# rvaser/rala

Measured on AMD Instinct MI355X. Metric: overlaps/sec (pile build + transitive reduction), higher is better.
Workload: dtype u16/u32 (+f64 compares)

## Files before the change

include/rala_hip.h:

```cpp
#ifndef RALA_HIP_H_
#define RALA_HIP_H_

#include <stddef.h>
#include <stdint.h>

#ifdef __cplusplus
extern "C" {
#endif

#define RALA_HIP_NO_READ 0xFFFFFFFFu

enum {
    RALA_HIP_OK = 0,
    RALA_HIP_EDEVICE = -1,
    RALA_HIP_EINVAL = -2,
    RALA_HIP_ECAPACITY = -3,
    RALA_HIP_EFILTERED = -4,
    RALA_HIP_ENOMEM = -5,
    RALA_HIP_ENOTAFILE = -6,
    RALA_HIP_ETOOLARGE = -7
};

enum { RALA_HIP_TYPE_X = 0, RALA_HIP_TYPE_A = 1, RALA_HIP_TYPE_B = 2, RALA_HIP_TYPE_AB = 3, RALA_HIP_TYPE_BA = 4 };

// ... 169 lines not shown

int rala_hip_get_valid(rala_hip_ctx* ctx, uint8_t* valid);
int rala_hip_get_piles(rala_hip_ctx* ctx, uint32_t* begin, uint32_t* end, uint16_t* median, uint16_t* p10,
                       uint8_t* alive);
int rala_hip_get_pile_data(rala_hip_ctx* ctx, uint64_t read, uint16_t* data);
int rala_hip_get_pile_row_digests(rala_hip_ctx* ctx, uint64_t* fnv, uint64_t* inside, uint64_t* outside);
int rala_hip_get_pile_rows_info(rala_hip_ctx* ctx, uint64_t* resident_bytes, uint64_t* rows_materialised);
int rala_hip_get_intervals(rala_hip_ctx* ctx, int kind, uint64_t* offsets, uint32_t* pairs, uint32_t* aux);
int rala_hip_get_overlaps(rala_hip_ctx* ctx, int which, uint64_t* n, uint32_t* src_index, uint32_t* a_begin,
                          uint32_t* a_end, uint32_t* b_begin, uint32_t* b_end, uint32_t* length, uint8_t* type);
int rala_hip_get_graph_size(rala_hip_ctx* ctx, uint64_t* n_nodes, uint64_t* n_edges);
int rala_hip_get_graph(rala_hip_ctx* ctx, uint32_t* node_read, uint32_t* src, uint32_t* dst, uint32_t* len,
                       uint8_t* marks);
int rala_hip_get_timings(rala_hip_ctx* ctx, rala_hip_timings* out);
int rala_hip_get_num_prefiltered(rala_hip_ctx* ctx, uint64_t* n);

#ifdef __cplusplus
}
#endif

#endif
```

rala_amd/csrc/kernels.h:

```cpp
#pragma once

#include <hip/hip_runtime.h>
#include <stdint.h>

#include "gzip_types.h"

namespace rala_hip {

constexpr uint32_t kPadL = 848;

enum : uint32_t {
    kErrRegionCapacity = 1u,
    kErrPoolCapacity = 2u,
    kErrRawCapacity = 4u,
};

struct Interval {
    uint32_t first, second;
    uint32_t aux;
};

struct PileArgs {
    const uint32_t* read_len;
    const uint64_t* pile_off;
// ... 250 lines not shown
    uint32_t* counts;
};
void launch_sens_split(const uint32_t* list, uint32_t bound, const uint32_t* n_dev, const SensSplitArgs& args, hipStream_t s);
void launch_status_clear(uint32_t* status, uint32_t bits, uint32_t* zero, hipStream_t s);
void launch_scatter_component_medians(const uint32_t* alive_reads, const uint8_t* touched, const uint16_t* cmed, uint32_t n_alive,
                                      uint16_t* out, hipStream_t s);
void launch_break_hills(const TailReads& R, uint32_t n_reads, hipStream_t s);
void launch_break_pits(const TailReads& R, const uint32_t* alive_reads, const uint8_t* touched, const uint16_t* comp_median,
                       uint32_t n_alive, hipStream_t s, const uint32_t* gate = nullptr);
void launch_retrim(const TailList& L, const TailReads& R, uint32_t promote, uint32_t round, uint32_t* dropped,
                   hipStream_t s, const uint32_t* gate = nullptr);
void launch_cc_edges(const TailList& L, const uint32_t* rank, uint32_t* edges, uint8_t* touched, uint32_t* label, uint32_t n_labels,
                     hipStream_t s);
void launch_refresh_types(const TailList& L, const TailReads& R, hipStream_t s);
hipError_t launch_tail_contain(const TailList& L, const TailReads& R, uint8_t* alive, uint32_t* const lists[6], uint32_t* zeroed21, uint32_t* const work[4],
                               uint32_t* base2, uint8_t* mark2, uint32_t* map, uint32_t* pack, uint32_t n_reads, uint32_t lds_limit, uint32_t debug_give_up, hipStream_t s);
void launch_count_zero_u8(const uint8_t* x, uint32_t n, uint32_t* out, hipStream_t s);
void launch_tail_init(const TailList& L, uint32_t n0, const TailReads& R, uint32_t* n_pits0, uint32_t n_reads, uint32_t* base2,
                      uint8_t* mark2, uint32_t* map, uint32_t* zero22, hipStream_t s);
struct ScanSpace;
bool launch_rank_pass(const uint8_t* alive, uint32_t* rank, uint32_t* alive_reads, uint32_t n_reads, ScanSpace& space, hipStream_t s);
bool launch_node_pass(const uint8_t* alive, uint32_t* node_rank, uint32_t* node_read, uint32_t* n_final, uint32_t n_reads,
                      ScanSpace& space, hipStream_t s);
bool launch_segment_pass(const TailList& L, const TailReads& R, uint32_t want_state, uint32_t want_round, uint32_t* base,
                         uint32_t* next, uint32_t* kept_item, const uint32_t* node_rank, uint32_t* e_src, uint32_t* e_dst,
                         uint32_t* e_len, ScanSpace& space, hipStream_t s);
bool launch_offsets_pass(const uint32_t* in, uint32_t* out, uint32_t* copy, uint32_t n, ScanSpace& space, hipStream_t s);
bool launch_pair_offsets_pass(const uint32_t* in0, const uint32_t* in1, uint32_t* out0, uint32_t* out1, uint32_t* totals, uint32_t n,
                              ScanSpace& space, hipStream_t s);

struct FixedPointList {
// ... 145 lines not shown
uint32_t gzip_segment_bytes();
uint32_t gzip_ring_symbols();
uint32_t gzip_crc_of_segments(const uint32_t* seg_crc, uint64_t text_n);
void launch_gzip_carry(uint16_t* sym, const uint8_t* text, uint64_t text_n, uint16_t* tmp, hipStream_t s);
uint32_t gzip_crc_register(const uint32_t* seg_crc, uint64_t text_n);
uint32_t gzip_crc_chain(const uint32_t* reg, const uint64_t* len, uint64_t n);
uint32_t gzip_crc_register_chain(const uint32_t* reg, const uint64_t* len, uint64_t n);

size_t scan_workspace_bytes(uint64_t n);
void launch_exclusive_scan(const uint32_t* in, uint32_t* out, uint64_t n, void* workspace, hipStream_t s);

void launch_tr_mark(const uint32_t* row_ptr, const uint32_t* adj_edge, const uint32_t* edge_src,
                    const uint32_t* edge_dst, const uint32_t* edge_len, uint32_t n_nodes, uint32_t first_edge,
                    uint32_t last_edge, uint8_t* marks, hipStream_t s);
void launch_tr_degree(const uint32_t* src, const uint32_t* dst, uint32_t n_nodes, uint32_t n_edges, uint32_t* deg,
                      uint32_t* bad, hipStream_t s);
void launch_tr_fill(const uint32_t* src, const uint32_t* dst, uint32_t n_nodes, uint32_t n_edges, uint32_t* cursor, uint32_t* adj,
                    hipStream_t s);
void launch_cc_init(uint32_t* label, uint32_t n, hipStream_t s);
void launch_cc_hook(const uint32_t* edges, uint32_t n_edges, uint32_t sample, uint32_t* label, uint32_t* changed,
                    hipStream_t s);
void launch_cc_compress(uint32_t* label, uint32_t n, hipStream_t s);
void launch_cc_compress_count(uint32_t* label, uint32_t n, const uint8_t* touched, uint32_t* size, hipStream_t s);
size_t component_median_workspace(uint32_t n);
void component_median_clear(void* tmp, uint32_t n, FillList& fills);
uint32_t* component_median_sizes(void* tmp, uint32_t n);
hipError_t launch_component_medians(const uint32_t* label, const uint8_t* touched, const uint32_t* alive_reads,
                                    const uint16_t* median, uint32_t n_alive, void* tmp, uint16_t* cmed, hipStream_t s);
void launch_tr_count(uint8_t* marks, uint32_t n_edges, uint32_t* n_pairs, hipStream_t s);

void launch_layout_step(uint32_t n, const double* x, const double* y, double* x_out, double* y_out,
                        const uint32_t* adj_off, const uint32_t* adj, double k, double t, hipStream_t s);

// ... 2 lines not shown
```

rala_amd/csrc/pipeline.hip:

```cpp
#include <hip/hip_runtime.h>
#include <stdio.h>
#include <stdlib.h>
#include <string.h>

#include <algorithm>
#include <chrono>
#include <numeric>

#include "context.h"
#include "scan_pass.h"
#include "stages.h"

using namespace rala_hip;


hipError_t rala_hip::d2h_small(rala_hip_ctx* ctx, void* dst, const void* src, size_t bytes, hipStream_t s) {
    if (ctx->p_stage.ensure(256) != hipSuccess || ctx->stage_used + bytes > 256 * sizeof(uint32_t) ||
        ctx->stage_pending.size() >= 16) {
        return hipMemcpyAsync(dst, src, bytes, hipMemcpyDeviceToHost, s);
    }
    char* at = (char*)ctx->p_stage.p + ctx->stage_used;
    const hipError_t e = hipMemcpyAsync(at, src, bytes, hipMemcpyDeviceToHost, s);
    if (e != hipSuccess) return e;
    ctx->stage_pending.push_back({dst, ctx->stage_used, bytes});
// ... 1192 lines not shown
    DevBuf<uint32_t>* B = ctx->d_tr;
    HIPCHECK(B[0].ensure(n_nodes + 2)); HIPCHECK(B[1].ensure(n_nodes + 2)); HIPCHECK(B[2].ensure(2 * (size_t)n_edges));
    HIPCHECK(ctx->d_tr_marks.ensure((size_t)n_edges + 8));
    HIPCHECK(ctx->d_scan_ws.ensure(scan_workspace_bytes((uint64_t)n_nodes + 2)));
    HIPCHECK(hipEventRecord(ctx->ev[10], s));
    FillList fills;
    fills.add(ctx->d_tr_marks.p, 0, ((size_t)n_edges + 7) & ~(size_t)3);
    fills.add(ctx->d_small.p + 2, 0, 8);
    fills.add(B[1].p, 0, (size_t)(n_nodes + 1) * 4);
    ScanSpace sp;
    {
        const int rc = scan_space(ctx, 1, n_nodes, sp, &fills);
        if (rc != RALA_HIP_OK) return rc;
    }
    HIPCHECK(fills.launch(s));
    launch_tr_degree(d_src, d_dst, n_nodes, n_edges, B[1].p, ctx->d_small.p + 2, s);
    HIPCHECK(B[3 + 3].ensure(n_nodes + 2));
    if (!launch_offsets_pass(B[1].p, B[0].p, B[6].p, n_nodes, sp, s)) return fail(ctx, RALA_HIP_EDEVICE, "scan space");
    launch_tr_fill(d_src, d_dst, n_nodes, n_edges, B[6].p, B[2].p, s);
    if (!comm) {
        launch_tr_mark(B[0].p, B[2].p, d_src, d_dst, d_len, n_nodes, 0, n_edges, ctx->d_tr_marks.p, s);
    } else {
        const uint64_t P = comm->world(), k = comm->rank();
        launch_tr_mark(B[0].p, B[2].p, d_src, d_dst, d_len, n_nodes, (uint32_t)(n_edges * k / P), (uint32_t)(n_edges * (k + 1) / P),
                       ctx->d_tr_marks.p, s);
        if (comm->all_reduce_u32((uint32_t*)ctx->d_tr_marks.p, ((size_t)n_edges + 3) / 4, ReduceOp::kSum, s) != 0) {
            ctx->err = std::string("all-reduce of the transitive marks: ") + comm->error();
            return RALA_HIP_EDEVICE;
        }
    }
    launch_tr_count(ctx->d_tr_marks.p, n_edges, ctx->d_small.p + 3, s);
    HIPCHECK(hipEventRecord(ctx->ev[11], s));
    uint32_t res[2] = {0, 0};
    HIPCHECK(d2h_small(ctx, res, ctx->d_small.p + 2, 8, s));
// ... 51 lines not shown
    else HIPCHECK(hipMemsetAsync(ctx->d_scan_state.p, 0, words * 8, ctx->stream));
    return RALA_HIP_OK;
}

int tail_components(rala_hip_ctx* ctx, const TailList& L, uint32_t n_alive, bool touched_cleared) {
    hipStream_t s = ctx->stream;
    const uint32_t M = L.n;
    if (!touched_cleared) {
        FillList fills;
        fills.add(ctx->d_touched.p, 0, n_alive);
        component_median_clear(ctx->d_med_tmp.p, n_alive, fills);
        HIPCHECK(fills.launch(s));
    }
    launch_cc_edges(L, ctx->d_rank.p, ctx->d_cc_edges.p, ctx->d_touched.p, ctx->d_cc_label.p, n_alive, s);
    for (int k = 0; k < 2; ++k) {
        launch_cc_hook(ctx->d_cc_edges.p, M, 1, ctx->d_cc_label.p, ctx->d_cc_flags.p + 7, s);
        launch_cc_compress(ctx->d_cc_label.p, n_alive, s);
    }
    launch_cc_hook(ctx->d_cc_edges.p, M, 0, ctx->d_cc_label.p, ctx->d_cc_flags.p + 7, s);
    launch_cc_compress_count(ctx->d_cc_label.p, n_alive, ctx->d_touched.p, component_median_sizes(ctx->d_med_tmp.p, n_alive), s);
    HIPCHECK(launch_component_medians(ctx->d_cc_label.p, ctx->d_touched.p, ctx->d_alive_reads.p, ctx->d_median.p, n_alive,
                                      ctx->d_med_tmp.p, ctx->d_cmed.p, s));
    return RALA_HIP_OK;
}

int gpu_tail_part_a(rala_hip_ctx* ctx) {
    hipStream_t s = ctx->stream;
    Trace trc;
    auto mark = [&](const char* what, size_t k = 0) {
        if (trc.on) { (void)stream_sync(ctx, s); trc(what, k); }
    };
// ... 32 lines not shown
    HIPCHECK(ctx->d_fp_pack.ensure(fixed_point_pack_words()));
    launch_tail_init(L, ctx->t_n0, R, ctx->d_n_pits0.p, n_reads, ctx->d_t_fin.p, ctx->d_t_mark.p, ctx->d_fp_map.p, ctx->d_counts.p + 9, s);
    if (!launch_rank_pass(ctx->d_alive.p, ctx->d_rank.p, ctx->d_alive_reads.p, n_reads, sp, s)) return fail(ctx, RALA_HIP_EDEVICE, "scan space");
    mark("tail: ranks", n_alive);

    HIPCHECK(ctx->d_counts.ensure(48));
    uint32_t* dropped = ctx->d_counts.p + 4;
    launch_break_hills(R, n_reads, s);
    if (ctx->lists_pending) {
        HIPCHECK(hipStreamWaitEvent(s, ctx->ev[3], 0));
        ctx->lists_pending = false;
    }
    launch_retrim(L, R, 0, 0, dropped, s);
    mark("tail: hills + retrim", M);

    uint32_t rounds = 0;
    for (;;) {
        const uint32_t batch = rounds == 0 ? 2u : 1u;
        for (uint32_t k = 0; k < batch; ++k) {
            if (rounds + k >= 255) return fail(ctx, RALA_HIP_EDEVICE, "chimera loop did not settle");
            const uint32_t* gate = k ? dropped + k - 1 : nullptr;
            FillList fills;
            fills.add(ctx->d_dirty.p, 0, n_reads);
            fills.add(ctx->d_touched.p, 0, n_alive);
            component_median_clear(ctx->d_med_tmp.p, n_alive, fills);
            if (k == 0) fills.add(dropped, 0, 2 * 4);
            HIPCHECK(fills.launch(s));
            const int rcc = tail_components(ctx, L, n_alive, true);
            if (rcc != RALA_HIP_OK) return rcc;
            launch_break_pits(R, ctx->d_alive_reads.p, ctx->d_touched.p, ctx->d_cmed.p, n_alive, s, gate);
            launch_retrim(L, R, 1, rounds + k, dropped + k, s, gate);
        }
        uint32_t d[2] = {0, 0};
        HIPCHECK(d2h_small(ctx, d, dropped, sizeof(d), s));
        HIPCHECK(stream_sync(ctx, s));
        mark("tail: pits + retrim", d[0] + d[1]);
        if (!d[0]) { rounds += 1; break; }
        rounds += batch;
        if (!d[batch - 1]) break;
    }
    ctx->t_rounds = rounds;
    if ((uint64_t)M * ((uint64_t)rounds + 2ull) >= 0xFFFFFFF0ull) {
        return fail(ctx, RALA_HIP_ETOOLARGE, "too many surviving overlaps for 32-bit list positions");
    }

    {
        uint32_t* const work[4] = {ctx->d_t_death[0].p, ctx->d_t_death[1].p, ctx->d_t_work[0].p, ctx->d_t_work[1].p};
        uint32_t* const lists[6] = {ctx->d_kill[0].p, ctx->d_kill[1].p, ctx->d_kill[2].p, ctx->d_kill2[0].p, ctx->d_kill2[1].p,
                                    ctx->d_kill2[2].p};
        HIPCHECK(launch_tail_contain(L, R, ctx->d_alive.p, lists, ctx->d_counts.p + 9, work, ctx->d_t_fin.p, ctx->d_t_mark.p, ctx->d_fp_map.p,
                                     ctx->d_fp_pack.p, n_reads, ctx->debug_fp_lds_limit, ctx->debug_fp_give_up, s));
    }
    mark("tail: containment scans", M);
    return RALA_HIP_OK;
}

int gpu_tail_part_b(rala_hip_ctx* ctx) {
    hipStream_t s = ctx->stream;
    Trace trc;
    auto mark = [&](const char* what, size_t k = 0) {
        if (trc.on) { (void)stream_sync(ctx, s); trc(what, k); }
    };
    const uint32_t n_reads = (uint32_t)ctx->n_reads;
    const uint32_t M = ctx->t_n0 + ctx->t_n1;
    const TailList L = tail_list(ctx);
    const TailReads R = tail_reads(ctx);
    const uint32_t n_seg = ctx->t_rounds + 1;
// ... 1765 lines not shown

int rala_hip_get_timings(rala_hip_ctx* ctx, rala_hip_timings* out) {
    if (!ctx || !out) return RALA_HIP_EINVAL;
    *out = ctx->tm;
    out->total_ms = ctx->tm.dedupe_ms + ctx->tm.bucket_ms + ctx->tm.pile_ms + ctx->tm.classify_ms + ctx->tm.death_ms +
                    ctx->tm.finish_ms + ctx->tm.tail_host_ms + ctx->tm.tr_ms;
    return RALA_HIP_OK;
}

int rala_hip_get_num_prefiltered(rala_hip_ctx* ctx, uint64_t* n) {
    if (!ctx || !n) return RALA_HIP_EINVAL;
    *n = ctx->n_prefiltered;
    return RALA_HIP_OK;
}

}
```

rala_amd/csrc/tail_kernels.hip:

```cpp
#include <hip/hip_runtime.h>

#include <algorithm>

#include "device_utils.h"
#include "geom.h"
#include "kernels.h"
#include "scan_pass.h"

namespace rala_hip {

namespace {

constexpr int kBlock = 256;
constexpr uint32_t kInf = 0xFFFFFFFFu;

inline dim3 grid_for(uint64_t n) { return dim3((unsigned)((n + kBlock - 1) / kBlock)); }

__device__ __forceinline__ bool dev_shrink(const TailReads& R, uint32_t r, uint32_t b, uint32_t e) {
    if (b > e || e - b < kMinRegion) { R.dirty[r] = 1; return false; }
    if (R.begin[r] != b || R.end[r] != e) R.dirty[r] = 1;
    R.begin[r] = b;
    R.end[r] = e;
    return true;
}
// ... 129 lines not shown
        if (m) {
            const uint32_t leader = (uint32_t)__ffsll((long long)m) - 1u;
            if (lane == leader) base = atomicAdd(s_cnt, (uint32_t)__popcll(m));
            base = (uint32_t)__shfl((int)base, (int)leader);
        }
        return mine ? base + (uint32_t)__popcll(m & ((1ull << lane) - 1ull)) : kInf;
    }
    __device__ void reserve(uint32_t* counter) const {
        __syncthreads();
        if (threadIdx.x == 0) *s_base = *s_cnt ? atomicAdd(counter, *s_cnt) : 0u;
        __syncthreads();
    }
};

__global__ __launch_bounds__(kContainBlock) void tail_contain_collect_kernel(TailList L, TailReads R, const uint8_t* __restrict__ alive,
                                                                             TailKillers K) {
    __shared__ uint32_t s_cnt[2], s_base[2];
    if (threadIdx.x < 2) s_cnt[threadIdx.x] = 0;
    __syncthreads();
    const BlockAppend app[2] = {{&s_cnt[0], &s_base[0]}, {&s_cnt[1], &s_base[1]}};
    uint32_t key[kCollectPer], target[kCollectPer], keeper[kCollectPer], slot[kCollectPer], cls[kCollectPer];
#pragma unroll
    for (uint32_t u = 0; u < kCollectPer; ++u) {
        const uint32_t k = (blockIdx.x * kCollectPer + u) * kContainBlock + threadIdx.x;
        bool killer = false;
        cls[u] = 0; key[u] = 0; target[u] = 0; keeper[u] = 0;
        if (k < L.n) {
            const uint8_t st = L.state[k];
            uint8_t t = L.type[k];
            if (st != 0 && t == 255) {
                const uint32_t a = L.a[k], b = L.b[k];
// ... 21 lines not shown
    app[1].reserve(&K.count[1]);
#pragma unroll
    for (uint32_t u = 0; u < kCollectPer; ++u) {
        if (slot[u] == kInf) continue;
        const uint32_t at = cls[u] ? L.n - 1u - (s_base[1] + slot[u]) : s_base[0] + slot[u];
        K.key[at] = key[u]; K.target[at] = target[u]; K.keeper[at] = keeper[u];
        K.mark[cls[u]][target[u]] = 1;
    }
}

__device__ __forceinline__ bool gone_before_second_scan(const uint8_t* alive, const uint32_t* base0, uint32_t r) {
    return !alive[r] || base0[r] != kInf;
}

template <int kClass>
__global__ __launch_bounds__(kBlock) void tail_contain_reduce_kernel(TailKillers K, uint32_t n_items, const uint8_t* __restrict__ alive) {
    __shared__ uint32_t s_cnt, s_base;
    const BlockAppend app = {&s_cnt, &s_base};
    const uint32_t n = K.count[kClass];
    uint32_t* base = K.base[kClass];
    for (uint32_t i0 = blockIdx.x * kBlock; i0 < n; i0 += gridDim.x * kBlock) {
        if (threadIdx.x == 0) s_cnt = 0;
        __syncthreads();
        const uint32_t i = i0 + threadIdx.x;
        bool conditional = false;
        uint32_t key = 0, target = 0, keeper = 0;
        if (i < n) {
            const uint32_t at = kClass ? n_items - 1u - i : i;
            key = K.key[at]; target = K.target[at]; keeper = K.keeper[at];
            const bool ok = kClass == 0 || !(gone_before_second_scan(alive, K.base[0], target) ||
                                             gone_before_second_scan(alive, K.base[0], keeper));
// ... 2 lines not shown
                else if (ld_past_l1(base + target) > key) atomicMin(base + target, key);
            }
        }
        const uint32_t slot = app.note(conditional);
        app.reserve(&K.count[2 + kClass]);
        if (conditional) {
            const uint32_t w = s_base + slot;
            K.c_key[w] = key; K.c_target[w] = target; K.c_keeper[w] = keeper;
        }
        __syncthreads();
    }
}

__global__ __launch_bounds__(kBlock) void tail_contain_apply_kernel(TailList L, const uint8_t* __restrict__ alive,
                                                                    const uint32_t* __restrict__ base0,
                                                                    const uint32_t* __restrict__ base1) {
    const uint32_t k = blockIdx.x * kBlock + threadIdx.x;
    if (k >= L.n) return;
    const uint8_t st = L.state[k];
    if (st == 0) return;
    const uint8_t t = L.type[k];
    bool drop = t == kTypeA || t == kTypeB;
    if (st == 2 && !drop) {
        const uint32_t a = L.a[k], b = L.b[k];
        drop = gone_before_second_scan(alive, base0, a) || gone_before_second_scan(alive, base0, b) || base1[a] < k || base1[b] < k;
    }
    if (drop) L.state[k] = 0;
}

__global__ __launch_bounds__(kBlock) void tail_contain_kill_kernel(TailKillers K, uint32_t n_items, uint8_t* alive) {
    const uint32_t n0 = K.count[0], n1 = K.count[1];
    for (uint32_t i = blockIdx.x * kBlock + threadIdx.x; i < n0 + n1; i += gridDim.x * kBlock) {
        const uint32_t target = K.target[i < n0 ? i : n_items - 1u - (i - n0)];
        if (K.base[0][target] != kInf || K.base[1][target] != kInf) alive[target] = 0;
    }
}

__global__ __launch_bounds__(kBlock) void tail_init_kernel(uint8_t* state, uint8_t* round, uint32_t n0, uint32_t m,
                                                           uint8_t* dirty, uint32_t* n_pits0, const uint32_t* n_pits,
                                                           uint32_t n_reads, uint32_t* base2, uint8_t* mark2, uint32_t* map, uint32_t* zero22) {
    const uint32_t k = blockIdx.x * kBlock + threadIdx.x;
    if (k < 22) zero22[k] = 0;
    if (k < n_reads) {
        base2[k] = kInf; base2[n_reads + k] = kInf; map[k] = kInf;
        mark2[k] = 0; mark2[n_reads + k] = 0;
// ... 115 lines not shown
    }
}
void launch_retrim(const TailList& L, const TailReads& R, uint32_t promote, uint32_t round, uint32_t* dropped,
                   hipStream_t s, const uint32_t* gate) {
    if (L.n) hipLaunchKernelGGL(retrim_kernel, grid_for(L.n), dim3(kBlock), 0, s, L, R, promote, round, dropped, gate);
}
void launch_cc_edges(const TailList& L, const uint32_t* rank, uint32_t* edges, uint8_t* touched, uint32_t* label, uint32_t n_labels,
                     hipStream_t s) {
    const uint32_t n = std::max<uint32_t>(L.n, n_labels);
    if (n) hipLaunchKernelGGL(cc_edges_kernel, grid_for(n), dim3(kBlock), 0, s, L, rank, edges, touched, label, n_labels);
}
void launch_refresh_types(const TailList& L, const TailReads& R, hipStream_t s) {
    if (L.n) hipLaunchKernelGGL(refresh_types_kernel, grid_for(L.n), dim3(kBlock), 0, s, L, R);
}
hipError_t launch_tail_contain(const TailList& L, const TailReads& R, uint8_t* alive, uint32_t* const lists[6], uint32_t* zeroed21, uint32_t* const work[4],
                               uint32_t* base2, uint8_t* mark2, uint32_t* map, uint32_t* pack, uint32_t n_reads, uint32_t lds_limit, uint32_t debug_give_up, hipStream_t s) {
    if (!L.n) return hipSuccess;
    TailKillers K;
    K.key = lists[0]; K.target = lists[1]; K.keeper = lists[2];
    K.c_key = lists[3]; K.c_target = lists[4]; K.c_keeper = lists[5];
    K.error = zeroed21; K.count = zeroed21 + 1;
    K.mark[0] = mark2; K.mark[1] = mark2 + n_reads;
    K.base[0] = base2; K.base[1] = base2 + n_reads;
    const uint32_t per_block = kCollectPer * kContainBlock;
    hipLaunchKernelGGL(tail_contain_collect_kernel, dim3((L.n + per_block - 1) / per_block), dim3(kContainBlock), 0, s, L, R,
                       (const uint8_t*)alive, K);
    for (int c = 0; c < 2; ++c) {
        if (c == 0) hipLaunchKernelGGL(tail_contain_reduce_kernel<0>, dim3(128), dim3(kBlock), 0, s, K, L.n, (const uint8_t*)alive);
        else hipLaunchKernelGGL(tail_contain_reduce_kernel<1>, dim3(128), dim3(kBlock), 0, s, K, L.n, (const uint8_t*)alive);
        const FixedPointList conditional = {K.c_key, K.c_target, K.c_keeper, K.count + 2 + c, lds_limit, debug_give_up};
        const hipError_t e = launch_fixed_point_finish(conditional, K.base[c], map, pack, work, zeroed21 + 5 + 8 * c, K.error, nullptr, s);
        if (e != hipSuccess) return e;
    }
    hipLaunchKernelGGL(tail_contain_apply_kernel, grid_for(L.n), dim3(kBlock), 0, s, L, (const uint8_t*)alive,
                       (const uint32_t*)K.base[0], (const uint32_t*)K.base[1]);
    hipLaunchKernelGGL(tail_contain_kill_kernel, dim3(128), dim3(kBlock), 0, s, K, L.n, alive);
    return hipGetLastError();
}
void launch_tail_init(const TailList& L, uint32_t n0, const TailReads& R, uint32_t* n_pits0, uint32_t n_reads, uint32_t* base2,
                      uint8_t* mark2, uint32_t* map, uint32_t* zero22, hipStream_t s) {
    const uint32_t n = std::max<uint32_t>(std::max<uint32_t>(L.n, n_reads), 22u);
    hipLaunchKernelGGL(tail_init_kernel, grid_for(n), dim3(kBlock), 0, s, L.state, L.round, n0, L.n, R.dirty, n_pits0, R.n_pits, n_reads,
                       base2, mark2, map, zero22);
}
bool launch_rank_pass(const uint8_t* alive, uint32_t* rank, uint32_t* alive_reads, uint32_t n_reads, ScanSpace& space, hipStream_t s) {
    return launch_scan_pass(n_reads, RankPass{alive, rank, alive_reads}, space, s);
}
bool launch_node_pass(const uint8_t* alive, uint32_t* node_rank, uint32_t* node_read, uint32_t* n_final, uint32_t n_reads,
                      ScanSpace& space, hipStream_t s) {
    return launch_scan_pass(n_reads, NodePass{alive, node_rank, node_read, n_final}, space, s);
}
// ... 29 lines not shown
```

rala_amd/csrc/tr_kernels.hip:

```cpp
#include <hip/hip_runtime.h>

#include "device_utils.h"
#include "geom.h"
#include "kernels.h"

namespace rala_hip {

namespace {

constexpr int kBlock = 256;

__global__ __launch_bounds__(kBlock) void tr_mark_kernel(const uint32_t* __restrict__ row_ptr,
                                                         const uint2* __restrict__ adj,
                                                         const uint32_t* __restrict__ esrc,
                                                         const uint32_t* __restrict__ edst,
                                                         const uint32_t* __restrict__ elen, uint32_t n_nodes,
                                                         uint32_t first_edge, uint32_t n_edges, uint8_t* marks) {
    const uint32_t e_ab = first_edge + blockIdx.x * kBlock + threadIdx.x;
    if (e_ab >= n_edges) return;
    const uint32_t a = esrc[e_ab], b = edst[e_ab];
    if (a >= n_nodes || b >= n_nodes) return;
    const uint32_t len_ab = elen[e_ab];
    const uint32_t a0 = row_ptr[a], a1 = row_ptr[a + 1];
    const uint32_t b0 = row_ptr[b], b1 = row_ptr[b + 1];
// ... 37 lines not shown
}

__global__ __launch_bounds__(kBlock) void tr_count_kernel(uint8_t* __restrict__ marks, uint32_t n_edges,
                                                          uint32_t* n_pairs) {
    __shared__ uint32_t tmp[kBlock / 64 + 1];
    uint32_t v = 0;
    for (uint32_t p = blockIdx.x * kBlock + threadIdx.x; 2 * p + 1 < n_edges; p += gridDim.x * kBlock) {
        if (marks[2 * p]) { marks[2 * p] = 1; marks[2 * p + 1] = 1; ++v; }
    }
    v = block_reduce<kBlock>(v, OpAdd(), 0u, tmp);
    if (threadIdx.x == 0 && v) atomicAdd(n_pairs, v);
}

__global__ __launch_bounds__(kBlock) void tr_degree_kernel(const uint32_t* __restrict__ src,
                                                           const uint32_t* __restrict__ dst, uint32_t n_nodes,
                                                           uint32_t n_edges, uint32_t* deg, uint32_t* bad) {
    const uint32_t e = blockIdx.x * kBlock + threadIdx.x;
    if (e >= n_edges) return;
    const uint32_t a = src[e], b = dst[e];
    if (a >= n_nodes || b >= n_nodes) { *bad = 1; return; }
    atomicAdd(&deg[a], 1u);
}

__global__ __launch_bounds__(kBlock) void tr_fill_kernel(const uint32_t* __restrict__ src, const uint32_t* __restrict__ dst,
                                                         uint32_t n_nodes, uint32_t n_edges, uint32_t* cursor, uint2* adj) {
    const uint32_t e = blockIdx.x * kBlock + threadIdx.x;
    if (e >= n_edges) return;
    const uint32_t a = src[e];
    if (a >= n_nodes) return;
    adj[atomicAdd(&cursor[a], 1u)] = make_uint2(e, dst[e]);
}

__global__ __launch_bounds__(kBlock) void cc_init_kernel(uint32_t* label, uint32_t n) {
    const uint32_t v = blockIdx.x * kBlock + threadIdx.x;
    if (v < n) label[v] = v;
}

__device__ __forceinline__ uint32_t cc_root(const uint32_t* label, uint32_t v) {
    uint32_t p = label[v];
    while (p != v) { v = p; p = label[v]; }
    return v;
}

__global__ __launch_bounds__(kBlock) void cc_hook_kernel(const uint32_t* __restrict__ edges, uint32_t n_edges,
                                                         uint32_t sample, uint32_t* label, uint32_t* changed) {
    const uint32_t e = blockIdx.x * kBlock + threadIdx.x;
    bool hooked = false;
    if (e < n_edges) {
        const uint32_t a = edges[2 * e], b = edges[2 * e + 1];
        if (a != b && (!sample || e < 2 || edges[2 * (e - 2)] != a)) {
            uint32_t ra = cc_root(label, a), rb = cc_root(label, b);
            while (ra != rb) {
                const uint32_t hi = ra > rb ? ra : rb, lo = ra > rb ? rb : ra;
                uint32_t old = __hip_atomic_load(&label[hi], __ATOMIC_RELAXED, __HIP_MEMORY_SCOPE_AGENT);
                if (old == hi) {
                    old = atomicMin(&label[hi], lo);
                    hooked = true;
                    if (old == hi) break;
                }
                ra = cc_root(label, old < lo ? old : lo);
                rb = cc_root(label, old < lo ? lo : old);
            }
        }
    }
    if (__ballot(hooked) != 0 && (threadIdx.x & 63) == 0) *changed = 1;
// ... 33 lines not shown
    if (threadIdx.x == 0) {
        uint32_t c = 0;
        for (int w = 0; w < kBlock / 64; ++w) c += s_cnt[w];
        atomicAdd(&size[shared], c);
    }
    if (t && !same) atomicAdd(&size[r], 1u);
}

}

void launch_cc_compress_count(uint32_t* label, uint32_t n, const uint8_t* touched, uint32_t* size, hipStream_t s) {
    if (n) hipLaunchKernelGGL(cc_compress_count_kernel, dim3((n + kBlock - 1) / kBlock), dim3(kBlock), 0, s, label, n, touched, size);
}

void launch_tr_degree(const uint32_t* src, const uint32_t* dst, uint32_t n_nodes, uint32_t n_edges, uint32_t* deg,
                      uint32_t* bad, hipStream_t s) {
    if (n_edges) {
        hipLaunchKernelGGL(tr_degree_kernel, dim3((n_edges + kBlock - 1) / kBlock), dim3(kBlock), 0, s, src, dst,
                           n_nodes, n_edges, deg, bad);
    }
}
void launch_tr_fill(const uint32_t* src, const uint32_t* dst, uint32_t n_nodes, uint32_t n_edges, uint32_t* cursor, uint32_t* adj,
                    hipStream_t s) {
    if (n_edges) {
        hipLaunchKernelGGL(tr_fill_kernel, dim3((n_edges + kBlock - 1) / kBlock), dim3(kBlock), 0, s, src, dst, n_nodes,
                           n_edges, cursor, (uint2*)adj);
    }
}
void launch_cc_init(uint32_t* label, uint32_t n, hipStream_t s) {
    if (n) hipLaunchKernelGGL(cc_init_kernel, dim3((n + kBlock - 1) / kBlock), dim3(kBlock), 0, s, label, n);
}
void launch_cc_hook(const uint32_t* edges, uint32_t n_edges, uint32_t sample, uint32_t* label, uint32_t* changed,
                    hipStream_t s) {
    if (n_edges) {
        hipLaunchKernelGGL(cc_hook_kernel, dim3((n_edges + kBlock - 1) / kBlock), dim3(kBlock), 0, s, edges, n_edges,
                           sample, label, changed);
    }
}
void launch_cc_compress(uint32_t* label, uint32_t n, hipStream_t s) {
    if (n) hipLaunchKernelGGL(cc_compress_kernel, dim3((n + kBlock - 1) / kBlock), dim3(kBlock), 0, s, label, n);
}
// ... 18 lines not shown
```

rala_amd/hip.py:

```python
import ctypes
import os

import numpy as np

from . import build as _build

TYPE_X, TYPE_A, TYPE_B, TYPE_AB, TYPE_BA = range(5)
NO_READ = 0xFFFFFFFF
MEM_HOST, MEM_DEVICE, MEM_HOST_ASYNC = 0, 1, 2

ERRORS = {0: "OK", -1: "EDEVICE", -2: "EINVAL", -3: "ECAPACITY", -4: "EFILTERED", -5: "ENOMEM", -6: "ENOTAFILE", -7: "ETOOLARGE"}

LIB_PATH = os.path.join(os.path.dirname(os.path.abspath(__file__)), "csrc", "librala_hip.so")

SYMBOLS = (
    "rala_hip_create", "rala_hip_destroy", "rala_hip_last_error", "rala_hip_set_option", "rala_hip_stream",
    "rala_hip_set_reads", "rala_hip_set_overlaps", "rala_hip_initialize", "rala_hip_construct",
    "rala_hip_remove_transitive_edges", "rala_hip_tr_mark", "rala_hip_get_valid", "rala_hip_get_piles",
    "rala_hip_get_pile_data", "rala_hip_get_pile_row_digests", "rala_hip_get_pile_rows_info", "rala_hip_get_intervals", "rala_hip_get_overlaps", "rala_hip_get_graph_size",
    "rala_hip_get_graph", "rala_hip_get_timings", "rala_hip_get_num_prefiltered",
    "rala_hip_dedupe", "rala_hip_emit_bound_tuples", "rala_hip_set_bound_tuples", "rala_hip_import_state",
    "rala_hip_emit_bound_tuples_bucketed", "rala_hip_get_device_state", "rala_hip_import_state_device",
    "rala_hip_bound_records_fit", "rala_hip_emit_bound_records_bucketed", "rala_hip_set_bound_records",
    "rala_hip_copy_device_state", "rala_hip_layout", "rala_hip_find_repetitive_hills",
    "rala_hip_mg_unique_id", "rala_hip_mg_local_group_create", "rala_hip_mg_local_group_destroy", "rala_hip_mg_create",
    "rala_hip_mg_create_contexts", "rala_hip_mg_join", "rala_hip_set_name_table", "rala_hip_set_overlaps_from_paf", "rala_hip_set_overlaps_from_mhap",
    "rala_hip_get_ingest_timings", "rala_hip_get_inflate_timings", "rala_hip_get_gzip_timings", "rala_hip_gzip_head", "rala_hip_gzip_chain", "rala_hip_gzip_chain_members", "rala_hip_gzip_find_members", "rala_hip_get_gzip_members", "rala_hip_bgzf_index", "rala_hip_get_overlap_columns", "rala_hip_tokenise_sensitive_paf",
    "rala_hip_mg_set_overlaps_from_paf", "rala_hip_mg_get_slice",
    "rala_hip_index_sequences", "rala_hip_get_sequence_index", "rala_hip_get_sequence_timings",
    "rala_hip_slice_sequences", "rala_hip_get_sequence_slice_info", "rala_hip_crc32_chain",
    "rala_hip_mg_destroy", "rala_hip_mg_last_error", "rala_hip_mg_set_reads", "rala_hip_mg_slice_cuts",
    "rala_hip_mg_set_overlaps", "rala_hip_mg_run", "rala_hip_mg_run_threads", "rala_hip_mg_context",
    "rala_hip_mg_owner_context",
    "rala_hip_mg_get_pile_data", "rala_hip_mg_get_pile_row_digests", "rala_hip_mg_get_timings",
)
# ... 83 lines not shown
        L.rala_hip_initialize.argtypes = [vp]
        L.rala_hip_construct.argtypes = [vp, ctypes.POINTER(OverlapsC), u64]
        L.rala_hip_remove_transitive_edges.argtypes = [vp, ctypes.POINTER(u32)]
        L.rala_hip_tr_mark.argtypes = [vp, u32, u32, vp, vp, vp, vp, ctypes.POINTER(u32)]
        L.rala_hip_get_valid.argtypes = [vp, vp]
        L.rala_hip_get_piles.argtypes = [vp, vp, vp, vp, vp, vp]
        L.rala_hip_get_pile_data.argtypes = [vp, u64, vp]
        L.rala_hip_get_pile_row_digests.argtypes = [vp, vp, vp, vp]
        L.rala_hip_get_pile_rows_info.argtypes = [vp, vp, vp]
        L.rala_hip_get_intervals.argtypes = [vp, i32, vp, vp, vp]
        L.rala_hip_get_overlaps.argtypes = [vp, i32, ctypes.POINTER(u64), vp, vp, vp, vp, vp, vp, vp]
        L.rala_hip_get_graph_size.argtypes = [vp, ctypes.POINTER(u64), ctypes.POINTER(u64)]
        L.rala_hip_get_graph.argtypes = [vp, vp, vp, vp, vp, vp]
        L.rala_hip_get_timings.argtypes = [vp, ctypes.POINTER(Timings)]
        L.rala_hip_get_num_prefiltered.argtypes = [vp, ctypes.POINTER(u64)]
        L.rala_hip_dedupe.argtypes = [vp]
        L.rala_hip_emit_bound_tuples.argtypes = [vp, vp]
        L.rala_hip_set_bound_tuples.argtypes = [vp, vp, u64, i32]
        L.rala_hip_import_state.argtypes = [vp] + [vp] * 11
        L.rala_hip_emit_bound_tuples_bucketed.argtypes = [vp, u32, vp, vp]
        L.rala_hip_get_device_state.argtypes = [vp, ctypes.POINTER(DeviceState)]
        L.rala_hip_import_state_device.argtypes = [vp, ctypes.POINTER(DeviceState)]
        L.rala_hip_copy_device_state.argtypes = [vp, ctypes.POINTER(DeviceState)]
        L.rala_hip_layout.argtypes = [vp, u32, vp, vp, vp, vp, u32, ctypes.c_double, ctypes.c_double, ctypes.c_double]
        L.rala_hip_find_repetitive_hills.argtypes = [vp, u64, u32, u32, ctypes.c_uint16, ctypes.c_uint16, ctypes.c_uint16]
        L.rala_hip_mg_unique_id.argtypes = [vp]
        L.rala_hip_mg_local_group_create.argtypes = [u32, ctypes.POINTER(vp)]
        L.rala_hip_mg_local_group_destroy.argtypes = [vp]
        L.rala_hip_mg_local_group_destroy.restype = None
        L.rala_hip_mg_create.argtypes = [i32, u32, u32, i32, vp, ctypes.POINTER(vp)]
# ... 379 lines not shown
        self._check(self.L.rala_hip_get_graph(self.h, d["node_read"].ctypes.data, d["src"].ctypes.data,
                                              d["dst"].ctypes.data, d["len"].ctypes.data,
                                              d["marked"].ctypes.data))
        return d

    def timings(self):
        t = Timings()
        self._check(self.L.rala_hip_get_timings(self.h, ctypes.byref(t)))
        return t.as_dict()

    def num_prefiltered(self):
        n = ctypes.c_uint64(0)
        self._check(self.L.rala_hip_get_num_prefiltered(self.h, ctypes.byref(n)))
        return int(n.value)


def slice_cuts(a_id, world, b_id=None):
    a = np.ascontiguousarray(a_id, dtype=np.uint32)
    b = None if b_id is None else np.ascontiguousarray(b_id, dtype=np.uint32)
    cuts = np.zeros(world + 1, dtype=np.uint64)
    rc = lib().rala_hip_mg_slice_cuts(a.ctypes.data if len(a) else None, b.ctypes.data if b is not None and len(b) else None,
                                      len(a), world, cuts.ctypes.data)
    if rc != 0:
        raise RalaHipError(rc, "slice_cuts")
    return [int(c) for c in cuts]


def unique_id():
    buf = ctypes.create_string_buffer(128)
    rc = lib().rala_hip_mg_unique_id(buf)
# ... 187 lines not shown
```

Baseline: 7.157 billion.

## Speculate containment scans ahead of retrim sync, slot-based CSR fill, cheap first hook

Containment scans are now enqueued speculatively before the host syncs on the first pits/retrim round. They are gated on a device flag, so the kernels exit early if further rounds are needed, and the scan is skipped later when it already ran. The transitive-reduction CSR fill records each edge's slot during the degree atomic, replacing the second atomic-cursor pass and the cursor copy in the offsets scan. The first connected-components hook pass uses a single relaxed load plus atomicMin instead of root chasing. A tail-rounds getter is added; the costs are extra edge-sized slot storage and possibly wasted speculative launches.

```diff
diff --git a/include/rala_hip.h b/include/rala_hip.h
--- a/include/rala_hip.h
+++ b/include/rala_hip.h
@@ -207,6 +207,7 @@
                        uint8_t* marks);
 int rala_hip_get_timings(rala_hip_ctx* ctx, rala_hip_timings* out);
 int rala_hip_get_num_prefiltered(rala_hip_ctx* ctx, uint64_t* n);
+int rala_hip_get_tail_rounds(rala_hip_ctx* ctx, uint32_t* rounds);
 
 #ifdef __cplusplus
 }
diff --git a/rala_amd/csrc/kernels.h b/rala_amd/csrc/kernels.h
--- a/rala_amd/csrc/kernels.h
+++ b/rala_amd/csrc/kernels.h
@@ -288,7 +288,8 @@
                      hipStream_t s);
 void launch_refresh_types(const TailList& L, const TailReads& R, hipStream_t s);
 hipError_t launch_tail_contain(const TailList& L, const TailReads& R, uint8_t* alive, uint32_t* const lists[6], uint32_t* zeroed21, uint32_t* const work[4],
-                               uint32_t* base2, uint8_t* mark2, uint32_t* map, uint32_t* pack, uint32_t n_reads, uint32_t lds_limit, uint32_t debug_give_up, hipStream_t s);
+                               uint32_t* base2, uint8_t* mark2, uint32_t* map, uint32_t* pack, uint32_t n_reads, uint32_t lds_limit, uint32_t debug_give_up, hipStream_t s,
+                               const uint32_t* closed = nullptr);
 void launch_count_zero_u8(const uint8_t* x, uint32_t n, uint32_t* out, hipStream_t s);
 void launch_tail_init(const TailList& L, uint32_t n0, const TailReads& R, uint32_t* n_pits0, uint32_t n_reads, uint32_t* base2,
                       uint8_t* mark2, uint32_t* map, uint32_t* zero22, hipStream_t s);
@@ -464,9 +465,9 @@
                     const uint32_t* edge_dst, const uint32_t* edge_len, uint32_t n_nodes, uint32_t first_edge,
                     uint32_t last_edge, uint8_t* marks, hipStream_t s);
 void launch_tr_degree(const uint32_t* src, const uint32_t* dst, uint32_t n_nodes, uint32_t n_edges, uint32_t* deg,
-                      uint32_t* bad, hipStream_t s);
-void launch_tr_fill(const uint32_t* src, const uint32_t* dst, uint32_t n_nodes, uint32_t n_edges, uint32_t* cursor, uint32_t* adj,
-                    hipStream_t s);
+                      uint32_t* slot, uint32_t* bad, hipStream_t s);
+void launch_tr_fill(const uint32_t* src, const uint32_t* dst, uint32_t n_nodes, uint32_t n_edges, const uint32_t* row_ptr,
+                    const uint32_t* slot, uint32_t* adj, hipStream_t s);
 void launch_cc_init(uint32_t* label, uint32_t n, hipStream_t s);
 void launch_cc_hook(const uint32_t* edges, uint32_t n_edges, uint32_t sample, uint32_t* label, uint32_t* changed,
                     hipStream_t s);
diff --git a/rala_amd/csrc/pipeline.hip b/rala_amd/csrc/pipeline.hip
--- a/rala_amd/csrc/pipeline.hip
+++ b/rala_amd/csrc/pipeline.hip
@@ -1230,10 +1230,10 @@
         if (rc != RALA_HIP_OK) return rc;
     }
     HIPCHECK(fills.launch(s));
-    launch_tr_degree(d_src, d_dst, n_nodes, n_edges, B[1].p, ctx->d_small.p + 2, s);
-    HIPCHECK(B[3 + 3].ensure(n_nodes + 2));
-    if (!launch_offsets_pass(B[1].p, B[0].p, B[6].p, n_nodes, sp, s)) return fail(ctx, RALA_HIP_EDEVICE, "scan space");
-    launch_tr_fill(d_src, d_dst, n_nodes, n_edges, B[6].p, B[2].p, s);
+    HIPCHECK(B[3 + 3].ensure(n_edges));
+    launch_tr_degree(d_src, d_dst, n_nodes, n_edges, B[1].p, B[6].p, ctx->d_small.p + 2, s);
+    if (!launch_offsets_pass(B[1].p, B[0].p, nullptr, n_nodes, sp, s)) return fail(ctx, RALA_HIP_EDEVICE, "scan space");
+    launch_tr_fill(d_src, d_dst, n_nodes, n_edges, B[0].p, B[6].p, B[2].p, s);
     if (!comm) {
         launch_tr_mark(B[0].p, B[2].p, d_src, d_dst, d_len, n_nodes, 0, n_edges, ctx->d_tr_marks.p, s);
     } else {
@@ -1315,7 +1315,7 @@
     }
     launch_cc_edges(L, ctx->d_rank.p, ctx->d_cc_edges.p, ctx->d_touched.p, ctx->d_cc_label.p, n_alive, s);
     for (int k = 0; k < 2; ++k) {
-        launch_cc_hook(ctx->d_cc_edges.p, M, 1, ctx->d_cc_label.p, ctx->d_cc_flags.p + 7, s);
+        launch_cc_hook(ctx->d_cc_edges.p, M, k == 0 ? 2u : 1u, ctx->d_cc_label.p, ctx->d_cc_flags.p + 7, s);
         launch_cc_compress(ctx->d_cc_label.p, n_alive, s);
     }
     launch_cc_hook(ctx->d_cc_edges.p, M, 0, ctx->d_cc_label.p, ctx->d_cc_flags.p + 7, s);
@@ -1378,6 +1378,16 @@
     launch_retrim(L, R, 0, 0, dropped, s);
     mark("tail: hills + retrim", M);
 
+    auto contain = [&](const uint32_t* closed) -> hipError_t {
+        uint32_t* const work[4] = {ctx->d_t_death[0].p, ctx->d_t_death[1].p, ctx->d_t_work[0].p, ctx->d_t_work[1].p};
+        uint32_t* const lists[6] = {ctx->d_kill[0].p, ctx->d_kill[1].p, ctx->d_kill[2].p, ctx->d_kill2[0].p, ctx->d_kill2[1].p,
+                                    ctx->d_kill2[2].p};
+        return launch_tail_contain(L, R, ctx->d_alive.p, lists, ctx->d_counts.p + 9, work, ctx->d_t_fin.p, ctx->d_t_mark.p, ctx->d_fp_map.p,
+                                   ctx->d_fp_pack.p, n_reads, ctx->debug_fp_lds_limit, ctx->debug_fp_give_up, s, closed);
+    };
+
+    const bool ahead = !trc.on && (uint64_t)M * 4ull < 0xFFFFFFF0ull;
+    bool contained = false;
     uint32_t rounds = 0;
     for (;;) {
         const uint32_t batch = rounds == 0 ? 2u : 1u;
@@ -1397,8 +1407,11 @@
         }
         uint32_t d[2] = {0, 0};
         HIPCHECK(d2h_small(ctx, d, dropped, sizeof(d), s));
+        const bool scans_ahead = rounds == 0 && ahead;
+        if (scans_ahead) HIPCHECK(contain(dropped + 1));
         HIPCHECK(stream_sync(ctx, s));
         mark("tail: pits + retrim", d[0] + d[1]);
+        if (scans_ahead && !d[1]) contained = true;
         if (!d[0]) { rounds += 1; break; }
         rounds += batch;
         if (!d[batch - 1]) break;
@@ -1407,14 +1420,7 @@
     if ((uint64_t)M * ((uint64_t)rounds + 2ull) >= 0xFFFFFFF0ull) {
         return fail(ctx, RALA_HIP_ETOOLARGE, "too many surviving overlaps for 32-bit list positions");
     }
-
-    {
-        uint32_t* const work[4] = {ctx->d_t_death[0].p, ctx->d_t_death[1].p, ctx->d_t_work[0].p, ctx->d_t_work[1].p};
-        uint32_t* const lists[6] = {ctx->d_kill[0].p, ctx->d_kill[1].p, ctx->d_kill[2].p, ctx->d_kill2[0].p, ctx->d_kill2[1].p,
-                                    ctx->d_kill2[2].p};
-        HIPCHECK(launch_tail_contain(L, R, ctx->d_alive.p, lists, ctx->d_counts.p + 9, work, ctx->d_t_fin.p, ctx->d_t_mark.p, ctx->d_fp_map.p,
-                                     ctx->d_fp_pack.p, n_reads, ctx->debug_fp_lds_limit, ctx->debug_fp_give_up, s));
-    }
+    if (!contained) HIPCHECK(contain(nullptr));
     mark("tail: containment scans", M);
     return RALA_HIP_OK;
 }
@@ -3210,4 +3216,10 @@
     return RALA_HIP_OK;
 }
 
-}
+int rala_hip_get_tail_rounds(rala_hip_ctx* ctx, uint32_t* rounds) {
+    if (!ctx || !rounds) return RALA_HIP_EINVAL;
+    *rounds = ctx->t_rounds;
+    return RALA_HIP_OK;
+}
+
+}
diff --git a/rala_amd/csrc/tail_kernels.hip b/rala_amd/csrc/tail_kernels.hip
--- a/rala_amd/csrc/tail_kernels.hip
+++ b/rala_amd/csrc/tail_kernels.hip
@@ -167,7 +167,8 @@
 };
 
 __global__ __launch_bounds__(kContainBlock) void tail_contain_collect_kernel(TailList L, TailReads R, const uint8_t* __restrict__ alive,
-                                                                             TailKillers K) {
+                                                                             TailKillers K, const uint32_t* closed) {
+    if (closed && *closed != 0) return;
     __shared__ uint32_t s_cnt[2], s_base[2];
     if (threadIdx.x < 2) s_cnt[threadIdx.x] = 0;
     __syncthreads();
@@ -219,7 +220,9 @@
 }
 
 template <int kClass>
-__global__ __launch_bounds__(kBlock) void tail_contain_reduce_kernel(TailKillers K, uint32_t n_items, const uint8_t* __restrict__ alive) {
+__global__ __launch_bounds__(kBlock) void tail_contain_reduce_kernel(TailKillers K, uint32_t n_items, const uint8_t* __restrict__ alive,
+                                                                     const uint32_t* closed) {
+    if (closed && *closed != 0) return;
     __shared__ uint32_t s_cnt, s_base;
     const BlockAppend app = {&s_cnt, &s_base};
     const uint32_t n = K.count[kClass];
@@ -252,7 +255,8 @@
 
 __global__ __launch_bounds__(kBlock) void tail_contain_apply_kernel(TailList L, const uint8_t* __restrict__ alive,
                                                                     const uint32_t* __restrict__ base0,
-                                                                    const uint32_t* __restrict__ base1) {
+                                                                    const uint32_t* __restrict__ base1, const uint32_t* closed) {
+    if (closed && *closed != 0) return;
     const uint32_t k = blockIdx.x * kBlock + threadIdx.x;
     if (k >= L.n) return;
     const uint8_t st = L.state[k];
@@ -266,7 +270,8 @@
     if (drop) L.state[k] = 0;
 }
 
-__global__ __launch_bounds__(kBlock) void tail_contain_kill_kernel(TailKillers K, uint32_t n_items, uint8_t* alive) {
+__global__ __launch_bounds__(kBlock) void tail_contain_kill_kernel(TailKillers K, uint32_t n_items, uint8_t* alive, const uint32_t* closed) {
+    if (closed && *closed != 0) return;
     const uint32_t n0 = K.count[0], n1 = K.count[1];
     for (uint32_t i = blockIdx.x * kBlock + threadIdx.x; i < n0 + n1; i += gridDim.x * kBlock) {
         const uint32_t target = K.target[i < n0 ? i : n_items - 1u - (i - n0)];
@@ -412,7 +417,8 @@
     if (L.n) hipLaunchKernelGGL(refresh_types_kernel, grid_for(L.n), dim3(kBlock), 0, s, L, R);
 }
 hipError_t launch_tail_contain(const TailList& L, const TailReads& R, uint8_t* alive, uint32_t* const lists[6], uint32_t* zeroed21, uint32_t* const work[4],
-                               uint32_t* base2, uint8_t* mark2, uint32_t* map, uint32_t* pack, uint32_t n_reads, uint32_t lds_limit, uint32_t debug_give_up, hipStream_t s) {
+                               uint32_t* base2, uint8_t* mark2, uint32_t* map, uint32_t* pack, uint32_t n_reads, uint32_t lds_limit, uint32_t debug_give_up, hipStream_t s,
+                               const uint32_t* closed) {
     if (!L.n) return hipSuccess;
     TailKillers K;
     K.key = lists[0]; K.target = lists[1]; K.keeper = lists[2];
@@ -422,17 +428,17 @@
     K.base[0] = base2; K.base[1] = base2 + n_reads;
     const uint32_t per_block = kCollectPer * kContainBlock;
     hipLaunchKernelGGL(tail_contain_collect_kernel, dim3((L.n + per_block - 1) / per_block), dim3(kContainBlock), 0, s, L, R,
-                       (const uint8_t*)alive, K);
+                       (const uint8_t*)alive, K, closed);
     for (int c = 0; c < 2; ++c) {
-        if (c == 0) hipLaunchKernelGGL(tail_contain_reduce_kernel<0>, dim3(128), dim3(kBlock), 0, s, K, L.n, (const uint8_t*)alive);
-        else hipLaunchKernelGGL(tail_contain_reduce_kernel<1>, dim3(128), dim3(kBlock), 0, s, K, L.n, (const uint8_t*)alive);
+        if (c == 0) hipLaunchKernelGGL(tail_contain_reduce_kernel<0>, dim3(128), dim3(kBlock), 0, s, K, L.n, (const uint8_t*)alive, closed);
+        else hipLaunchKernelGGL(tail_contain_reduce_kernel<1>, dim3(128), dim3(kBlock), 0, s, K, L.n, (const uint8_t*)alive, closed);
         const FixedPointList conditional = {K.c_key, K.c_target, K.c_keeper, K.count + 2 + c, lds_limit, debug_give_up};
         const hipError_t e = launch_fixed_point_finish(conditional, K.base[c], map, pack, work, zeroed21 + 5 + 8 * c, K.error, nullptr, s);
         if (e != hipSuccess) return e;
     }
     hipLaunchKernelGGL(tail_contain_apply_kernel, grid_for(L.n), dim3(kBlock), 0, s, L, (const uint8_t*)alive,
-                       (const uint32_t*)K.base[0], (const uint32_t*)K.base[1]);
-    hipLaunchKernelGGL(tail_contain_kill_kernel, dim3(128), dim3(kBlock), 0, s, K, L.n, alive);
+                       (const uint32_t*)K.base[0], (const uint32_t*)K.base[1], closed);
+    hipLaunchKernelGGL(tail_contain_kill_kernel, dim3(128), dim3(kBlock), 0, s, K, L.n, alive, closed);
     return hipGetLastError();
 }
 void launch_tail_init(const TailList& L, uint32_t n0, const TailReads& R, uint32_t* n_pits0, uint32_t n_reads, uint32_t* base2,
diff --git a/rala_amd/csrc/tr_kernels.hip b/rala_amd/csrc/tr_kernels.hip
--- a/rala_amd/csrc/tr_kernels.hip
+++ b/rala_amd/csrc/tr_kernels.hip
@@ -75,21 +75,24 @@
 
 __global__ __launch_bounds__(kBlock) void tr_degree_kernel(const uint32_t* __restrict__ src,
                                                            const uint32_t* __restrict__ dst, uint32_t n_nodes,
-                                                           uint32_t n_edges, uint32_t* deg, uint32_t* bad) {
+                                                           uint32_t n_edges, uint32_t* deg, uint32_t* __restrict__ slot,
+                                                           uint32_t* bad) {
     const uint32_t e = blockIdx.x * kBlock + threadIdx.x;
     if (e >= n_edges) return;
     const uint32_t a = src[e], b = dst[e];
     if (a >= n_nodes || b >= n_nodes) { *bad = 1; return; }
-    atomicAdd(&deg[a], 1u);
+    slot[e] = atomicAdd(&deg[a], 1u);
 }
 
 __global__ __launch_bounds__(kBlock) void tr_fill_kernel(const uint32_t* __restrict__ src, const uint32_t* __restrict__ dst,
-                                                         uint32_t n_nodes, uint32_t n_edges, uint32_t* cursor, uint2* adj) {
+                                                         uint32_t n_nodes, uint32_t n_edges,
+                                                         const uint32_t* __restrict__ row_ptr,
+                                                         const uint32_t* __restrict__ slot, uint2* __restrict__ adj) {
     const uint32_t e = blockIdx.x * kBlock + threadIdx.x;
     if (e >= n_edges) return;
-    const uint32_t a = src[e];
-    if (a >= n_nodes) return;
-    adj[atomicAdd(&cursor[a], 1u)] = make_uint2(e, dst[e]);
+    const uint32_t a = src[e], b = dst[e];
+    if (a >= n_nodes || b >= n_nodes) return;
+    adj[row_ptr[a] + slot[e]] = make_uint2(e, b);
 }
 
 __global__ __launch_bounds__(kBlock) void cc_init_kernel(uint32_t* label, uint32_t n) {
@@ -109,7 +112,14 @@
     bool hooked = false;
     if (e < n_edges) {
         const uint32_t a = edges[2 * e], b = edges[2 * e + 1];
-        if (a != b && (!sample || e < 2 || edges[2 * (e - 2)] != a)) {
+        const bool takes_part = a != b && (!sample || e < 2 || edges[2 * (e - 2)] != a);
+        if (takes_part && sample == 2) {
+            const uint32_t hi = a > b ? a : b, lo = a > b ? b : a;
+            if (__hip_atomic_load(&label[hi], __ATOMIC_RELAXED, __HIP_MEMORY_SCOPE_AGENT) > lo) {
+                atomicMin(&label[hi], lo);
+                hooked = true;
+            }
+        } else if (takes_part) {
             uint32_t ra = cc_root(label, a), rb = cc_root(label, b);
             while (ra != rb) {
                 const uint32_t hi = ra > rb ? ra : rb, lo = ra > rb ? rb : ra;
@@ -173,17 +183,17 @@
 }
 
 void launch_tr_degree(const uint32_t* src, const uint32_t* dst, uint32_t n_nodes, uint32_t n_edges, uint32_t* deg,
-                      uint32_t* bad, hipStream_t s) {
+                      uint32_t* slot, uint32_t* bad, hipStream_t s) {
     if (n_edges) {
         hipLaunchKernelGGL(tr_degree_kernel, dim3((n_edges + kBlock - 1) / kBlock), dim3(kBlock), 0, s, src, dst,
-                           n_nodes, n_edges, deg, bad);
-    }
-}
-void launch_tr_fill(const uint32_t* src, const uint32_t* dst, uint32_t n_nodes, uint32_t n_edges, uint32_t* cursor, uint32_t* adj,
-                    hipStream_t s) {
+                           n_nodes, n_edges, deg, slot, bad);
+    }
+}
+void launch_tr_fill(const uint32_t* src, const uint32_t* dst, uint32_t n_nodes, uint32_t n_edges, const uint32_t* row_ptr,
+                    const uint32_t* slot, uint32_t* adj, hipStream_t s) {
     if (n_edges) {
         hipLaunchKernelGGL(tr_fill_kernel, dim3((n_edges + kBlock - 1) / kBlock), dim3(kBlock), 0, s, src, dst, n_nodes,
-                           n_edges, cursor, (uint2*)adj);
+                           n_edges, row_ptr, slot, (uint2*)adj);
     }
 }
 void launch_cc_init(uint32_t* label, uint32_t n, hipStream_t s) {
diff --git a/rala_amd/hip.py b/rala_amd/hip.py
--- a/rala_amd/hip.py
+++ b/rala_amd/hip.py
@@ -18,7 +18,7 @@
     "rala_hip_set_reads", "rala_hip_set_overlaps", "rala_hip_initialize", "rala_hip_construct",
     "rala_hip_remove_transitive_edges", "rala_hip_tr_mark", "rala_hip_get_valid", "rala_hip_get_piles",
     "rala_hip_get_pile_data", "rala_hip_get_pile_row_digests", "rala_hip_get_pile_rows_info", "rala_hip_get_intervals", "rala_hip_get_overlaps", "rala_hip_get_graph_size",
-    "rala_hip_get_graph", "rala_hip_get_timings", "rala_hip_get_num_prefiltered",
+    "rala_hip_get_graph", "rala_hip_get_timings", "rala_hip_get_num_prefiltered", "rala_hip_get_tail_rounds",
     "rala_hip_dedupe", "rala_hip_emit_bound_tuples", "rala_hip_set_bound_tuples", "rala_hip_import_state",
     "rala_hip_emit_bound_tuples_bucketed", "rala_hip_get_device_state", "rala_hip_import_state_device",
     "rala_hip_bound_records_fit", "rala_hip_emit_bound_records_bucketed", "rala_hip_set_bound_records",
@@ -132,6 +132,7 @@
         L.rala_hip_get_graph.argtypes = [vp, vp, vp, vp, vp, vp]
         L.rala_hip_get_timings.argtypes = [vp, ctypes.POINTER(Timings)]
         L.rala_hip_get_num_prefiltered.argtypes = [vp, ctypes.POINTER(u64)]
+        L.rala_hip_get_tail_rounds.argtypes = [vp, ctypes.POINTER(u32)]
         L.rala_hip_dedupe.argtypes = [vp]
         L.rala_hip_emit_bound_tuples.argtypes = [vp, vp]
         L.rala_hip_set_bound_tuples.argtypes = [vp, vp, u64, i32]
@@ -541,6 +542,11 @@
         self._check(self.L.rala_hip_get_num_prefiltered(self.h, ctypes.byref(n)))
         return int(n.value)
 
+    def tail_rounds(self):
+        n = ctypes.c_uint32(0)
+        self._check(self.L.rala_hip_get_tail_rounds(self.h, ctypes.byref(n)))
+        return int(n.value)
+
 
 def slice_cuts(a_id, world, b_id=None):
     a = np.ascontiguousarray(a_id, dtype=np.uint32)
```

Measured after the change: 7.146 billion. About the same (-0.2%).
